# MarinerQ/npf_GWwaveform

Measured on AMD Instinct MI355X. Metric: waveform target-points/sec (train step), higher is better.
Workload: dtype f32 (every contraction of the step: fp32 operands as three exact bf16 terms, six v_mfma_f32_16x16x32_bf16 per product group, f32 accumulation -- f32 results, DESIGN.md 3.1 / 3.2; the 1-4-wide first / last layers: f32 FMAs); 1 GPU; BASELINE config 2: AttnCNP scaledot, r=256, 4-layer xy-encoder/decoder, 256 context / 1024 target points, 256 tasks per GPU (256 global), fp32 train step (fwd+loss+bwd+allreduce+Adam); tasks_per_gpu=256, global_tasks=256, context_points=256, target_points=1024, r_dim=256, n_params=799588, parallelism=dp1, hip_graph=True

## Files before the change

### npf_gwwaveform_amd/csrc/wgrad_kernel.hip

```cpp
#include "npf_common.hpp"

namespace npf {

constexpr int kWgThreads = 1024;
constexpr int kWgWaves = kWgThreads / 64;
constexpr int kWgMaxF = 256;
constexpr int kQRows = kWgMaxF / 4;
constexpr int kMaxJobs = 16;

struct WgradJobs {
  npf_wgrad_job_t job[kMaxJobs];
  int32_t first_wg[kMaxJobs + 1];
  int32_t n_jobs;
  int32_t n_tasks;
  int32_t tiles_per_task;
  int32_t pad;
  int64_t part_off[kMaxJobs];
};

__device__ __forceinline__ void wg_dma16(const float* src, float* lds_dst_wave_uniform) {
  __builtin_amdgcn_global_load_lds((const __attribute__((address_space(1))) void*)src,
                                   (__attribute__((address_space(3))) void*)lds_dst_wave_uniform, 16, 0, 0);
}

typedef __bf16 bf16x4 __attribute__((ext_vector_type(4)));
typedef __bf16 bf16x8w __attribute__((ext_vector_type(8)));
typedef __bf16 bf16x2v __attribute__((ext_vector_type(2)));
typedef float f32x2v __attribute__((ext_vector_type(2)));

__device__ __forceinline__ bf16x4 pack4_bf16(float a, float b, float c, float d) {
  const bf16x2v lo = __builtin_convertvector((f32x2v{a, b}), bf16x2v), hi = __builtin_convertvector((f32x2v{c, d}), bf16x2v);
  bf16x4 r;
  r[0] = lo[0]; r[1] = lo[1]; r[2] = hi[0]; r[3] = hi[1];
  return r;
}

__device__ __forceinline__ int wg_s0(int blk) { return 4 * (blk >> 1) + (blk & 1); }

__device__ __forceinline__ void operand16(const float* img, bool fmt16, int blk, int i, int g, int t2, bf16x4 (&op)[4],
                                          bool want_sum, f32x4& dsum) {
  if (!fmt16) {
    f32x4 q[4];
    const unsigned lbase = (unsigned)(size_t)(const __attribute__((address_space(3))) float*)img + (16 * blk + i) * 512;
#pragma unroll
    for (int jj = 0; jj < 4; ++jj) {
      const int c = 16 * t2 + 4 * g + jj;
      asm volatile("ds_read_b128 %0, %1" : "=v"(q[jj]) : "v"(lbase + ((c ^ i) << 4)));
    }
    asm volatile("s_waitcnt lgkmcnt(0)" : "+v"(q[0]), "+v"(q[1]), "+v"(q[2]), "+v"(q[3]));
    if (want_sum) dsum += (q[0] + q[1]) + (q[2] + q[3]);
#pragma unroll
    for (int m = 0; m < 4; ++m) op[m] = pack4_bf16(q[0][m], q[1][m], q[2][m], q[3][m]);
  } else {
    typedef unsigned u32x2 __attribute__((ext_vector_type(2)));
    const int q = i >> 2, p = i & 3;
    const int row0 = 4 * (wg_s0(blk) + 2 * (p >> 1));
    const int point = 16 * t2 + 4 * g + q;
    const unsigned base = (unsigned)(size_t)(const __attribute__((address_space(3))) float*)img + 8u * (p & 1);
    u32x2 r[4];
#pragma unroll
    for (int m = 0; m < 4; ++m) {
      const int row = row0 + m;
      asm volatile("ds_read_b64_tr_b16 %0, %1" : "=v"(r[m]) : "v"(base + row * 512 + ((point ^ (row & 15)) << 4)));
    }
    asm volatile("s_waitcnt lgkmcnt(0)" : "+v"(r[0]), "+v"(r[1]), "+v"(r[2]), "+v"(r[3]));
#pragma unroll
    for (int m = 0; m < 4; ++m) {
      op[m] = __builtin_bit_cast(bf16x4, r[m]);
    }
    if (want_sum) {
      f32x4 sm;
#pragma unroll
      for (int m = 0; m < 4; ++m)
        sm[m] = (__builtin_bit_cast(float, r[m][0] << 16) + __builtin_bit_cast(float, r[m][0] & 0xffff0000u)) +
                (__builtin_bit_cast(float, r[m][1] << 16) + __builtin_bit_cast(float, r[m][1] & 0xffff0000u));
      dsum += sm;
    }
  }
}

__device__ __forceinline__ int wg_feature(bool fmt16, int blk, int i, int m) {
  if (!fmt16) return 4 * (16 * blk + i) + m;
  return 32 * (wg_s0(blk) + 2 * (i >> 3)) + 16 * ((i >> 2) & 1) + 4 * m + (i & 3);
}
__device__ __forceinline__ bool wg_block_active(bool fmt16, int blk, int Fp) {
  return fmt16 ? 32 * wg_s0(blk) < Fp : 64 * blk < Fp;
}

template <bool BF16>
__global__ __launch_bounds__(kWgThreads, 4) void wgrad_kernel(const WgradJobs J, float* __restrict__ partials) {
  __shared__ __attribute__((aligned(16))) float lds[2 * 2 * kQRows * 128];
  constexpr int kOp = kQRows * 128;

  int j = 0;
  while (j + 1 < J.n_jobs && (int)blockIdx.x >= J.first_wg[j + 1]) ++j;
  const npf_wgrad_job_t& job = J.job[j];
  const int split = blockIdx.x - J.first_wg[j];
  const int n_split = J.first_wg[j + 1] - J.first_wg[j];
  const int Np = ((job.N + 31) >> 5) * 32, Kp = ((job.K + 31) >> 5) * 32;
  const long total_tiles = (long)J.n_tasks * J.tiles_per_task;
  long t0, t1;
  int tstride = 1;
  if (job.per_task) {
    t0 = (long)split * J.tiles_per_task;
    t1 = t0 + J.tiles_per_task;
  } else {
    t0 = split;
    t1 = total_tiles;
    tstride = n_split;
  }

  const int tid = threadIdx.x, lane = tid & 63;
  const int i = lane & 15, g = lane >> 4;
  const int wave = __builtin_amdgcn_readfirstlane(tid >> 6);
  const bool wide_rows = ((Kp + 63) >> 6) < ((Np + 63) >> 6);
  const int rg = wide_rows ? (wave & 3) : (wave >> 2);
  const int cg = wide_rows ? (wave >> 2) : (wave & 3);
  const bool act = wg_block_active(BF16 && (job.accumulate & NPF_WGRAD_DZ16) != 0, rg, Np) &&
                   wg_block_active(BF16 && (job.accumulate & NPF_WGRAD_A16) != 0, cg, Kp);

  for (int x = tid; x < 2 * 2 * kOp; x += kWgThreads) lds[x] = 0.f;

  const f32x4 zero4 = {0.f, 0.f, 0.f, 0.f};
  f32x4 acc[4][4];
#pragma unroll
  for (int m = 0; m < 4; ++m)
#pragma unroll
    for (int n = 0; n < 4; ++n) acc[m][n] = zero4;
  f32x4 dbacc = zero4;

  const unsigned dma_lane = 4u * (unsigned)((lane >> 5) * 128 + (((lane & 31) ^ ((2 * wave + (lane >> 5)) & 15)) << 2));
  const char* dz_base = (const char*)job.dZ;
  const char* a_base = (const char*)job.A;
  asm volatile("" : "+s"(dz_base), "+s"(a_base));
  const bool z16 = BF16 && (job.accumulate & NPF_WGRAD_DZ16) != 0, a16 = BF16 && (job.accumulate & NPF_WGRAD_A16) != 0;
  const int zsh = z16 ? 4 : 3, ash = a16 ? 4 : 3;
  const int Zf = job.ldz > 0 ? job.ldz : Np, Af = job.lda > 0 ? job.lda : Kp;
  auto tile_dma = [&](long t, float* buf) {
    const char* zsrc = dz_base + (((size_t)t * Zf) << (10 - zsh));
    const char* asrc = a_base + (((size_t)t * Af) << (10 - ash));
    for (int q = wave; q < (Np >> zsh); q += kWgWaves)
      wg_dma16((const float*)(zsrc + (size_t)q * 1024 + (size_t)dma_lane), buf + q * 256);
    for (int q = wave; q < (Kp >> ash); q += kWgWaves)
      wg_dma16((const float*)(asrc + (size_t)q * 1024 + (size_t)dma_lane), buf + kOp + q * 256);
  };

  [[maybe_unused]] const bool dual = z16 && a16;
  const long tstep = (BF16 && dual) ? 2 * (long)tstride : (long)tstride;
  auto step_dma = [&](long t, float* buf) {
    tile_dma(t, buf);
    if constexpr (BF16) {
      if (dual && t + tstride < t1) tile_dma(t + tstride, buf + kOp / 2);
    }
  };

  __syncthreads();
  if (t0 < t1 && !(BF16 && dual)) step_dma(t0, lds);

  unsigned za_l[4], ab_l[4];
  {
    const unsigned l0 = (unsigned)(size_t)(const __attribute__((address_space(3))) float*)lds;
#pragma unroll
    for (int t = 0; t < 4; ++t) {
      const unsigned lanepart = (((t ^ (i >> 2)) << 2) | (g ^ (i & 3))) << 4;
      za_l[t] = l0 + (16 * rg + i) * 512 + lanepart;
      ab_l[t] = l0 + kOp * 4 + (16 * cg + i) * 512 + lanepart;
    }
  }

  if constexpr (BF16) {
    if (dual) {
      const int pw = (wave < (Np >> zsh) ? 1 : 0) + (wave < (Kp >> ash) ? 1 : 0);
      auto slot_of = [&](long n) { return lds + ((n >> 1) & 1) * 2 * kOp + (n & 1) * (kOp / 2); };
      const long n_tiles = t0 < t1 ? (t1 - t0 + tstride - 1) / tstride : 0;
      for (long n = 0; n < 3 && n < n_tiles; ++n) tile_dma(t0 + n * tstride, slot_of(n));
      for (long n = 0; n < n_tiles; ++n) {
        const long younger = (n_tiles - 1 - n) < 2 ? (n_tiles - 1 - n) : 2;
        const int allow = (int)younger * pw;
        if (allow >= 4) asm volatile("s_waitcnt vmcnt(4)" ::: "memory");
        else if (allow >= 2) asm volatile("s_waitcnt vmcnt(2)" ::: "memory");
        else if (allow >= 1) asm volatile("s_waitcnt vmcnt(1)" ::: "memory");
        else asm volatile("s_waitcnt vmcnt(0)" ::: "memory");
        __builtin_amdgcn_s_barrier();
        if (n + 3 < n_tiles) tile_dma(t0 + (n + 3) * tstride, slot_of(n + 3));
        if (act) {
          const float* zimg = slot_of(n);
          const float* aimg = zimg + kOp;
          bf16x4 am[2][4], bn[2][4];
          f32x4 none = zero4;
          int iv = i, gv = g;
          asm volatile("" : "+v"(iv), "+v"(gv));
#pragma unroll
          for (int t2 = 0; t2 < 2; ++t2) {
            operand16(zimg, true, rg, iv, gv, t2, am[t2], cg == 0, dbacc);
            operand16(aimg, true, cg, iv, gv, t2, bn[t2], false, none);
          }
          bf16x8w a8[4], b8[4];
#pragma unroll
          for (int m = 0; m < 4; ++m) {
            a8[m] = __builtin_shufflevector(am[0][m], am[1][m], 0, 1, 2, 3, 4, 5, 6, 7);
            b8[m] = __builtin_shufflevector(bn[0][m], bn[1][m], 0, 1, 2, 3, 4, 5, 6, 7);
          }
#pragma unroll
          for (int m = 0; m < 4; ++m)
#pragma unroll
            for (int n2 = 0; n2 < 4; ++n2)
              acc[m][n2] = __builtin_amdgcn_mfma_f32_16x16x32_bf16(a8[m], b8[n2], acc[m][n2], 0, 0, 0);
        }
      }
      t0 = t1;
    }
  }
  int cur = 1;
  for (long t = t0; t < t1; t += tstep) {
    cur ^= 1;
    __syncthreads();
    if (t + tstep < t1) step_dma(t + tstep, lds + (cur ^ 1) * 2 * kOp);
    [[maybe_unused]] const unsigned boff = cur * 2 * kOp * 4;
    if constexpr (BF16) {
      const int nsub = (dual && t + tstride < t1) ? 2 : 1;
#pragma unroll 1
      for (int u = 0; act && u < nsub; ++u) {
        const float* zimg = lds + cur * 2 * kOp + u * (kOp / 2);
        const float* aimg = zimg + kOp;
#pragma unroll
        for (int t2 = 0; t2 < 2; ++t2) {
          bf16x4 am[4], bn[4];
          f32x4 none = zero4;
          int iv = i, gv = g;
          asm volatile("" : "+v"(iv), "+v"(gv));
          operand16(zimg, z16, rg, iv, gv, t2, am, cg == 0, dbacc);
          operand16(aimg, a16, cg, iv, gv, t2, bn, false, none);
#pragma unroll
          for (int m = 0; m < 4; ++m)
#pragma unroll
            for (int n2 = 0; n2 < 4; ++n2)
              acc[m][n2] = __builtin_amdgcn_mfma_f32_16x16x16bf16_1k(am[m], bn[n2], acc[m][n2], 0, 0, 0);
        }
      }
    } else if (act) {
      f32x4 fa[2], fb[2];
      asm volatile("ds_read_b128 %0, %2\n\tds_read_b128 %1, %3"
                   : "=&v"(fa[0]), "=&v"(fb[0])
                   : "v"(za_l[0] + boff), "v"(ab_l[0] + boff));
#pragma unroll
      for (int s = 0; s < 8; ++s) {
        const int c = s & 1, n = c ^ 1;
        if (s + 1 < 8) {
          asm volatile("s_waitcnt lgkmcnt(0)\n\tds_read_b128 %0, %4 offset:%6\n\tds_read_b128 %1, %5 offset:%6"
                       : "=&v"(fa[n]), "=&v"(fb[n]), "+v"(fa[c]), "+v"(fb[c])
                       : "v"(za_l[(s + 1) & 3] + boff), "v"(ab_l[(s + 1) & 3] + boff), "n"(((s + 1) >> 2) * 256));
        } else {
          asm volatile("s_waitcnt lgkmcnt(0)" : "+v"(fa[c]), "+v"(fb[c]));
        }
        if (cg == 0) dbacc += fa[c];
#pragma unroll
        for (int m = 0; m < 4; ++m)
#pragma unroll
          for (int n2 = 0; n2 < 4; ++n2)
            acc[m][n2] = __builtin_amdgcn_mfma_f32_16x16x4f32(fa[c][m], fb[c][n2], acc[m][n2], 0, 0, 0);
      }
    }
  }

  if (act) {
    int col[4];
#pragma unroll
    for (int n = 0; n < 4; ++n) col[n] = wg_feature(a16, cg, i, n);
    if (job.per_task) {
      const int Ko = job.ldo > 0 ? job.ldo : Kp;
      float* out = job.dW + (size_t)split * ((size_t)(Np >> 5) * Ko * 32);
#pragma unroll
      for (int m = 0; m < 4; ++m)
#pragma unroll
        for (int e = 0; e < 4; ++e) {
          const int row = wg_feature(z16, rg, 4 * g + e, m);
          if (row >= Np) continue;
          float* rbase = out + (size_t)(row >> 5) * (Ko >> 2) * 128 + (row & 31) * 4;
          if (!a16) {
            if (col[0] < Kp) {
              f32x4 v;
#pragma unroll
              for (int n = 0; n < 4; ++n) v[n] = acc[m][n][e];
              float* dst = rbase + (size_t)(col[0] >> 2) * 128;
              if (job.accumulate & NPF_WGRAD_ACCUMULATE) v += *(const f32x4*)dst;
              *(f32x4*)dst = v;
            }
          } else {
#pragma unroll
            for (int n = 0; n < 4; ++n)
              if (col[n] < Kp) {
                float* dst = rbase + (size_t)(col[n] >> 2) * 128 + (col[n] & 3);
                *dst = (job.accumulate & NPF_WGRAD_ACCUMULATE) ? *dst + acc[m][n][e] : acc[m][n][e];
              }
          }
        }
    } else {
      float* part = partials + J.part_off[j] + (size_t)split * ((size_t)Np * Kp + Np);
#pragma unroll
      for (int m = 0; m < 4; ++m)
#pragma unroll
        for (int e = 0; e < 4; ++e) {
          const int row = wg_feature(z16, rg, 4 * g + e, m);
          if (row >= Np) continue;
          if (!a16) {
            if (col[0] < Kp) {
              f32x4 v;
#pragma unroll
              for (int n = 0; n < 4; ++n) v[n] = acc[m][n][e];
              *(f32x4*)(part + (size_t)row * Kp + col[0]) = v;
            }
          } else {
#pragma unroll
            for (int n = 0; n < 4; ++n)
              if (col[n] < Kp) part[(size_t)row * Kp + col[n]] = acc[m][n][e];
          }
        }
      if (cg == 0) {
#pragma unroll
        for (int m = 0; m < 4; ++m) {
          dbacc[m] += __shfl_xor(dbacc[m], 16);
          dbacc[m] += __shfl_xor(dbacc[m], 32);
        }
        if (g == 0) {
          if (!z16) {
            if (wg_feature(false, rg, i, 0) < Np) *(f32x4*)(part + (size_t)Np * Kp + wg_feature(false, rg, i, 0)) = dbacc;
          } else {
#pragma unroll
            for (int m = 0; m < 4; ++m)
              if (wg_feature(true, rg, i, m) < Np) part[(size_t)Np * Kp + wg_feature(true, rg, i, m)] = dbacc[m];
          }
        }
      }
    }
  }
}

constexpr int kXThreads = 512;
constexpr int kXWaves = kXThreads / 64;

typedef float f32x8v __attribute__((ext_vector_type(8)));
struct X6Terms { bf16x8w t[3]; };

__device__ __forceinline__ unsigned x6_cvt_pk(float a, float b) {
  unsigned r;
  asm("v_cvt_pk_bf16_f32 %0, %1, %2" : "=v"(r) : "v"(a), "v"(b));
  return r;
}
__device__ __forceinline__ X6Terms x6_split(f32x8v v) {
  typedef unsigned u32x4v __attribute__((ext_vector_type(4)));
  u32x4v t0, t1, t2;
#pragma unroll
  for (int p = 0; p < 4; ++p) {
    const float a = v[2 * p], b = v[2 * p + 1];
    const unsigned h = x6_cvt_pk(a, b);
    const float ra = a - __builtin_bit_cast(float, h << 16), rb = b - __builtin_bit_cast(float, h & 0xffff0000u);
    const unsigned m = x6_cvt_pk(ra, rb);
    const float la = ra - __builtin_bit_cast(float, m << 16), lb = rb - __builtin_bit_cast(float, m & 0xffff0000u);
    t0[p] = h;
    t1[p] = m;
    t2[p] = x6_cvt_pk(la, lb);
  }
  X6Terms o;
  o.t[0] = __builtin_bit_cast(bf16x8w, t0);
  o.t[1] = __builtin_bit_cast(bf16x8w, t1);
  o.t[2] = __builtin_bit_cast(bf16x8w, t2);
  return o;
}

struct X6Raw { f32x4 q[8]; };
__device__ __forceinline__ void x6_issue(const unsigned (&ad)[4], X6Raw& r) {
  asm volatile("ds_read_b128 %0, %8\n\tds_read_b128 %1, %9\n\tds_read_b128 %2, %10\n\tds_read_b128 %3, %11\n\t"
               "ds_read_b128 %4, %8 offset:256\n\tds_read_b128 %5, %9 offset:256\n\t"
               "ds_read_b128 %6, %10 offset:256\n\tds_read_b128 %7, %11 offset:256"
               : "=&v"(r.q[0]), "=&v"(r.q[1]), "=&v"(r.q[2]), "=&v"(r.q[3]), "=&v"(r.q[4]), "=&v"(r.q[5]), "=&v"(r.q[6]),
                 "=&v"(r.q[7])
               : "v"(ad[0]), "v"(ad[1]), "v"(ad[2]), "v"(ad[3]));
}
struct X6Feat { float v[8]; };
template <int SEL>
__device__ __forceinline__ void x6_issue_feat(const unsigned (&ad)[4], X6Feat& r) {
  asm volatile("ds_read_b32 %0, %8 offset:%12\n\tds_read_b32 %1, %9 offset:%12\n\t"
               "ds_read_b32 %2, %10 offset:%12\n\tds_read_b32 %3, %11 offset:%12\n\t"
               "ds_read_b32 %4, %8 offset:%13\n\tds_read_b32 %5, %9 offset:%13\n\t"
               "ds_read_b32 %6, %10 offset:%13\n\tds_read_b32 %7, %11 offset:%13"
               : "=&v"(r.v[0]), "=&v"(r.v[1]), "=&v"(r.v[2]), "=&v"(r.v[3]), "=&v"(r.v[4]), "=&v"(r.v[5]), "=&v"(r.v[6]),
                 "=&v"(r.v[7])
               : "v"(ad[0]), "v"(ad[1]), "v"(ad[2]), "v"(ad[3]), "n"(SEL * 8192), "n"(SEL * 8192 + 256));
}
template <int N>
__device__ __forceinline__ void x6_wait_feat(X6Feat& r) {
  asm volatile("s_waitcnt lgkmcnt(%8)"
               : "+v"(r.v[0]), "+v"(r.v[1]), "+v"(r.v[2]), "+v"(r.v[3]), "+v"(r.v[4]), "+v"(r.v[5]), "+v"(r.v[6]), "+v"(r.v[7])
               : "n"(N));
}
__device__ __forceinline__ X6Terms x6_terms_of(const X6Feat& r) {
  return x6_split(f32x8v{r.v[0], r.v[1], r.v[2], r.v[3], r.v[4], r.v[5], r.v[6], r.v[7]});
}
__device__ __forceinline__ void x6_wait(X6Raw& r) {
  asm volatile("s_waitcnt lgkmcnt(0)"
               : "+v"(r.q[0]), "+v"(r.q[1]), "+v"(r.q[2]), "+v"(r.q[3]), "+v"(r.q[4]), "+v"(r.q[5]), "+v"(r.q[6]), "+v"(r.q[7]));
}
__device__ __forceinline__ X6Terms x6_terms_of(const X6Raw& r, int f) {
  const f32x8v v = {r.q[0][f], r.q[1][f], r.q[2][f], r.q[3][f], r.q[4][f], r.q[5][f], r.q[6][f], r.q[7][f]};
  return x6_split(v);
}

__global__ __launch_bounds__(kXThreads, 1) void wgrad_x6_kernel(const WgradJobs J, float* __restrict__ partials) {
  __shared__ __attribute__((aligned(16))) float lds[2 * 2 * kQRows * 128];
  constexpr int kOp = kQRows * 128;

  int j = 0;
  while (j + 1 < J.n_jobs && (int)blockIdx.x >= J.first_wg[j + 1]) ++j;
  const npf_wgrad_job_t& job = J.job[j];
  const int split = blockIdx.x - J.first_wg[j];
  const int n_split = J.first_wg[j + 1] - J.first_wg[j];
  const int Np = ((job.N + 31) >> 5) * 32, Kp = ((job.K + 31) >> 5) * 32;
  const long total_tiles = (long)J.n_tasks * J.tiles_per_task;
  long t0, t1;
  int tstride = 1;
  if (job.per_task) {
    t0 = (long)split * J.tiles_per_task;
    t1 = t0 + J.tiles_per_task;
  } else {
    t0 = split;
    t1 = total_tiles;
    tstride = n_split;
  }

  const int tid = threadIdx.x, lane = tid & 63;
  const int i = lane & 15, g = lane >> 4;
  const int wave = __builtin_amdgcn_readfirstlane(tid >> 6);
  const int rg = wave >> 1, cp = wave & 1;
  const bool act_r = 64 * rg < Np && 128 * cp < Kp;
  const int n_steps = !act_r ? 0 : (64 * (2 * cp + 1) < Kp ? 8 : 4);

  for (int x = tid; x < 2 * 2 * kOp; x += kXThreads) lds[x] = 0.f;

  const f32x4 zero4 = {0.f, 0.f, 0.f, 0.f};
  f32x4 acc[2][4][4];
#pragma unroll
  for (int c = 0; c < 2; ++c)
#pragma unroll
    for (int m = 0; m < 4; ++m)
#pragma unroll
      for (int n = 0; n < 4; ++n) acc[c][m][n] = zero4;
  f32x4 dbacc = zero4;

  const unsigned dma_lane = 4u * (unsigned)((lane >> 5) * 128 + (((lane & 31) ^ ((2 * wave + (lane >> 5)) & 15)) << 2));
  const char* dz_base = (const char*)job.dZ;
  const char* a_base = (const char*)job.A;
  asm volatile("" : "+s"(dz_base), "+s"(a_base));
  const int Zf = job.ldz > 0 ? job.ldz : Np, Af = job.lda > 0 ? job.lda : Kp;
  auto tile_dma = [&](long t, float* buf) {
    const char* zsrc = dz_base + (size_t)t * Zf * 128;
    const char* asrc = a_base + (size_t)t * Af * 128;
    for (int q = wave; q < (Np >> 3); q += kXWaves)
      wg_dma16((const float*)(zsrc + (size_t)q * 1024 + (size_t)dma_lane), buf + q * 256);
    for (int q = wave; q < (Kp >> 3); q += kXWaves)
      wg_dma16((const float*)(asrc + (size_t)q * 1024 + (size_t)dma_lane), buf + kOp + q * 256);
  };

  __syncthreads();
  if (t0 < t1) tile_dma(t0, lds);

  int cur = 1;
  for (long t = t0; t < t1; t += tstride) {
    cur ^= 1;
    __syncthreads();
    const bool dma_next = t + tstride < t1;
    float* nbuf = lds + (cur ^ 1) * 2 * kOp;
    if (n_steps == 0) {
      if (dma_next) tile_dma(t + tstride, nbuf);
      continue;
    }
    const char* zsrc_n = dz_base + (size_t)(t + tstride) * Zf * 128 + (size_t)dma_lane;
    const char* asrc_n = a_base + (size_t)(t + tstride) * Af * 128 + (size_t)dma_lane;
    int iv = i, gv = g;
    asm volatile("" : "+v"(iv), "+v"(gv));
    unsigned za[4], zb[4];
    {
      const unsigned l0 = (unsigned)(size_t)(const __attribute__((address_space(3))) float*)lds + cur * 2 * kOp * 4;
#pragma unroll
      for (int jj = 0; jj < 4; ++jj) {
        const unsigned lanepart = (unsigned)(((4 * gv + jj) ^ iv) << 4);
        za[jj] = l0 + (16 * rg + iv) * 512 + lanepart;
        zb[jj] = l0 + kOp * 4 + (32 * cp + iv) * 512 + lanepart;
      }
    }
    X6Raw ra;
    x6_issue(za, ra);
    x6_wait(ra);
    if (cp == 0) dbacc += ((ra.q[0] + ra.q[1]) + (ra.q[2] + ra.q[3])) + ((ra.q[4] + ra.q[5]) + (ra.q[6] + ra.q[7]));
    X6Terms fa[4];
#pragma unroll
    for (int m = 0; m < 4; ++m) fa[m] = x6_terms_of(ra, m);
    const unsigned pi4 = (unsigned)((iv >> 3) & 1) << 3;
    auto feat_addr = [&](int n2, unsigned (&ad)[4]) {
#pragma unroll
      for (int jj = 0; jj < 4; ++jj) ad[jj] = zb[jj] + ((4u * (unsigned)n2) ^ pi4);
    };
    X6Feat raw[2];
    {
      unsigned ad[4];
      feat_addr(0, ad);
      x6_issue_feat<0>(ad, raw[0]);
      feat_addr(1, ad);
      x6_issue_feat<0>(ad, raw[1]);
    }
    x6_wait_feat<8>(raw[0]);
    X6Terms fb = x6_terms_of(raw[0]);
#pragma unroll
    for (int k = 0; k < 8; ++k) {
      const int c = k >> 2, n2 = k & 3;
      if (dma_next) {
        const int q = wave + kXWaves * (k & 3);
        if (k < 4) {
          if (q < (Np >> 3)) wg_dma16((const float*)(zsrc_n + (size_t)q * 1024), nbuf + q * 256);
        } else {
          if (q < (Kp >> 3)) wg_dma16((const float*)(asrc_n + (size_t)q * 1024), nbuf + kOp + q * 256);
        }
      }
      if (k + 2 < 8) {
        unsigned ad[4];
        feat_addr((k + 2) & 3, ad);
        if (k + 2 < 4) x6_issue_feat<0>(ad, raw[k & 1]);
        else x6_issue_feat<1>(ad, raw[k & 1]);
      }
      X6Terms fb_next;
      if (k + 1 < 8) {
        if (k + 2 < 8) x6_wait_feat<8>(raw[(k + 1) & 1]);
        else x6_wait_feat<0>(raw[(k + 1) & 1]);
        fb_next = x6_terms_of(raw[(k + 1) & 1]);
      }
#pragma unroll
      for (int m = 0; m < 4; ++m) {
        f32x4 a = acc[c][m][n2];
        a = __builtin_amdgcn_mfma_f32_16x16x32_bf16(fa[m].t[2], fb.t[0], a, 0, 0, 0);
        a = __builtin_amdgcn_mfma_f32_16x16x32_bf16(fa[m].t[0], fb.t[2], a, 0, 0, 0);
        a = __builtin_amdgcn_mfma_f32_16x16x32_bf16(fa[m].t[1], fb.t[1], a, 0, 0, 0);
        a = __builtin_amdgcn_mfma_f32_16x16x32_bf16(fa[m].t[1], fb.t[0], a, 0, 0, 0);
        a = __builtin_amdgcn_mfma_f32_16x16x32_bf16(fa[m].t[0], fb.t[1], a, 0, 0, 0);
        a = __builtin_amdgcn_mfma_f32_16x16x32_bf16(fa[m].t[0], fb.t[0], a, 0, 0, 0);
        acc[c][m][n2] = a;
      }
      if (k + 1 < 8) {
#pragma unroll
        for (int q = 0; q < 24; ++q) {
          __builtin_amdgcn_sched_group_barrier(0x008, 1, 0);
          __builtin_amdgcn_sched_group_barrier(0x002, 2, 0);
        }
        fb = fb_next;
      }
    }
  }

#pragma unroll
  for (int c = 0; c < 2; ++c) {
    if (4 * c >= n_steps) continue;
    const int cg = 2 * cp + c;
    const int col0 = 4 * (16 * cg + i);
    if (job.per_task) {
      const int Ko = job.ldo > 0 ? job.ldo : Kp;
      float* out = job.dW + (size_t)split * ((size_t)(Np >> 5) * Ko * 32);
#pragma unroll
      for (int m = 0; m < 4; ++m)
#pragma unroll
        for (int e = 0; e < 4; ++e) {
          const int row = 4 * (16 * rg + 4 * g + e) + m;
          if (row >= Np || col0 >= Kp) continue;
          f32x4 v;
#pragma unroll
          for (int n = 0; n < 4; ++n) v[n] = (i & 8) ? acc[c][m][n ^ 2][e] : acc[c][m][n][e];
          float* dst = out + (size_t)(row >> 5) * (Ko >> 2) * 128 + (row & 31) * 4 + (size_t)(col0 >> 2) * 128;
          if (job.accumulate & NPF_WGRAD_ACCUMULATE) v += *(const f32x4*)dst;
          *(f32x4*)dst = v;
        }
    } else {
      float* part = partials + J.part_off[j] + (size_t)split * ((size_t)Np * Kp + Np);
#pragma unroll
      for (int m = 0; m < 4; ++m)
#pragma unroll
        for (int e = 0; e < 4; ++e) {
          const int row = 4 * (16 * rg + 4 * g + e) + m;
          if (row >= Np || col0 >= Kp) continue;
          f32x4 v;
#pragma unroll
          for (int n = 0; n < 4; ++n) v[n] = (i & 8) ? acc[c][m][n ^ 2][e] : acc[c][m][n][e];
          *(f32x4*)(part + (size_t)row * Kp + col0) = v;
        }
    }
  }
  if (!job.per_task && n_steps > 0 && cp == 0) {
    float* part = partials + J.part_off[j] + (size_t)split * ((size_t)Np * Kp + Np);
#pragma unroll
    for (int m = 0; m < 4; ++m) {
      dbacc[m] += __shfl_xor(dbacc[m], 16);
      dbacc[m] += __shfl_xor(dbacc[m], 32);
    }
    if (g == 0 && 4 * (16 * rg + i) < Np) *(f32x4*)(part + (size_t)Np * Kp + 4 * (16 * rg + i)) = dbacc;
  }
}

constexpr int kHRow = 576;
constexpr int kHTerm = 16 * kHRow;
constexpr int kHBuf = 2 * 3 * kHTerm;
typedef unsigned h16_u32x2 __attribute__((ext_vector_type(2)));
typedef unsigned h16_u32x4 __attribute__((ext_vector_type(4)));
typedef float f32x16v __attribute__((ext_vector_type(16)));

__global__ __launch_bounds__(512, 1) void wgrad_h16_kernel(const WgradJobs J, float* __restrict__ partials) {
  __shared__ __attribute__((aligned(16))) char lds[2 * kHBuf];
  int j = 0;
  while (j + 1 < J.n_jobs && (int)blockIdx.x >= J.first_wg[j + 1]) ++j;
  const npf_wgrad_job_t& job = J.job[j];
  const int split = blockIdx.x - J.first_wg[j];
  const int n_split = J.first_wg[j + 1] - J.first_wg[j];
  constexpr int Np = 256, Kp = 256;
  const long total_tiles = (long)J.n_tasks * J.tiles_per_task;
  long t0, t1;
  int tstride = 1;
  if (job.per_task) {
    t0 = (long)split * J.tiles_per_task;
    t1 = t0 + J.tiles_per_task;
  } else {
    t0 = split;
    t1 = total_tiles;
    tstride = n_split;
  }
  const long n_half = t1 > t0 ? 2 * ((t1 - t0 + tstride - 1) / tstride) : 0;

  const int tid = threadIdx.x, lane = tid & 63;
  const int wave = __builtin_amdgcn_readfirstlane(tid >> 6);
  const int rg = wave >> 1, cp = wave & 1;
  const int p_lo = lane & 3, q_ld = (lane >> 2) & 3, p_hi = lane >> 4;
  const int pt_ld = 4 * p_hi + p_lo;
  const int Zf = job.ldz > 0 ? job.ldz : Np, Af = job.lda > 0 ? job.lda : Kp;
  const char* dz_base = (const char*)job.dZ;
  const char* a_base = (const char*)job.A;
  const unsigned ld_lane = (unsigned)(((8 * wave + q_ld) * 32 + pt_ld) * 16);
  auto tile_of = [&](long h) { return t0 + (h >> 1) * tstride; };
  auto load_piece = [&](long h, int v) -> f32x4 {
    const long t = tile_of(h);
    const unsigned off = ld_lane + (unsigned)(h & 1) * 256u + (unsigned)(v & 1) * 2048u;
    const char* src = (v < 2 ? dz_base + (size_t)t * Zf * 128 : a_base + (size_t)t * Af * 128) + off;
    return *(const f32x4*)src;
  };
  const unsigned lds0 = (unsigned)(size_t)(__attribute__((address_space(3))) char*)lds;
  const unsigned st_lane = (unsigned)(pt_ld * kHRow + (8 * wave + q_ld) * 8);
  auto split_store1 = [&](const f32x4& x, int v, unsigned buf) {
    h16_u32x2 t[3];
#pragma unroll
    for (int pr = 0; pr < 2; ++pr) {
      const float a = x[2 * pr], b = x[2 * pr + 1];
      const unsigned h = x6_cvt_pk(a, b);
      const float ra = a - __builtin_bit_cast(float, h << 16), rb = b - __builtin_bit_cast(float, h & 0xffff0000u);
      const unsigned m = x6_cvt_pk(ra, rb);
      const float la = ra - __builtin_bit_cast(float, m << 16), lb = rb - __builtin_bit_cast(float, m & 0xffff0000u);
      t[0][pr] = h;
      t[1][pr] = m;
      t[2][pr] = x6_cvt_pk(la, lb);
    }
    const unsigned ad = lds0 + buf * kHBuf + (v >> 1) * 3 * kHTerm + st_lane + (v & 1) * 32;
    asm volatile("ds_write_b64 %0, %1\n\tds_write_b64 %0, %2 offset:%4\n\tds_write_b64 %0, %3 offset:%5"
                 :
                 : "v"(ad), "v"(t[0]), "v"(t[1]), "v"(t[2]), "n"(kHTerm), "n"(2 * kHTerm)
                 : "memory");
  };
  const int gq = lane >> 4, q_rd = (lane >> 2) & 3, p_rd = lane & 3;
  const unsigned rd_lane = (unsigned)((8 * (gq >> 1) + q_rd) * kHRow + (16 * (gq & 1) + 4 * p_rd) * 2);
  typedef short h16_s16x4 __attribute__((ext_vector_type(4)));
  typedef short h16_s16x8 __attribute__((ext_vector_type(8)));
  typedef __attribute__((address_space(3))) h16_s16x4 h16_lds_s16x4;
  struct Frag { h16_s16x8 v; };
  auto frag = [&](unsigned buf, int operand, int term, int feat0, Frag& f) {
    const char* ad = lds + buf * kHBuf + (operand * 3 + term) * kHTerm + rd_lane + (unsigned)feat0 * 2;
    const h16_s16x4 lo = __builtin_amdgcn_ds_read_tr16_b64_v4i16((h16_lds_s16x4*)ad);
    const h16_s16x4 hi = __builtin_amdgcn_ds_read_tr16_b64_v4i16((h16_lds_s16x4*)(ad + 4 * kHRow));
    f.v = __builtin_shufflevector(lo, hi, 0, 1, 2, 3, 4, 5, 6, 7);
  };
  auto op8 = [](const Frag& f) { return __builtin_bit_cast(bf16x8w, f.v); };

  f32x16v acc[2][4];
#pragma unroll
  for (int i = 0; i < 2; ++i)
#pragma unroll
    for (int c = 0; c < 4; ++c)
#pragma unroll
      for (int r = 0; r < 16; ++r) acc[i][c][r] = 0.f;
  f32x4 dbacc[2] = {f32x4{0.f, 0.f, 0.f, 0.f}, f32x4{0.f, 0.f, 0.f, 0.f}};

  f32x4 raw[4];
  auto body = [&](long h) {
    const unsigned buf = (unsigned)(h & 1);
    const float live = h + 1 < n_half ? 1.f : 0.f;
    const long h2 = h + 2 < n_half ? h + 2 : (n_half > 0 ? n_half - 1 : 0);
    Frag fa[2][3], fb[2][3];
#pragma unroll
    for (int i = 0; i < 2; ++i)
#pragma unroll
      for (int t = 0; t < 3; ++t) frag(buf, 0, t, 64 * rg + 32 * i, fa[i][t]);
#pragma unroll
    for (int t = 0; t < 3; ++t) frag(buf, 1, t, 128 * cp, fb[0][t]);
#pragma unroll
    for (int c = 0; c < 4; ++c) {
      const int cb = c & 1;
      if (c + 1 < 4) {
#pragma unroll
        for (int t = 0; t < 3; ++t) frag(buf, 1, t, 128 * cp + 32 * (c + 1), fb[cb ^ 1][t]);
      }
#define HMM(I, TA, TB) \
  acc[I][c] = __builtin_amdgcn_mfma_f32_32x32x16_bf16(op8(fa[I][TA]), op8(fb[cb][TB]), acc[I][c], 0, 0, 0)
      HMM(0, 2, 0);
      HMM(1, 2, 0);
      HMM(0, 0, 2);
      HMM(1, 0, 2);
      HMM(0, 1, 1);
      HMM(1, 1, 1);
      HMM(0, 1, 0);
      HMM(1, 1, 0);
      HMM(0, 0, 1);
      HMM(1, 0, 1);
      HMM(0, 0, 0);
      HMM(1, 0, 0);
#undef HMM
      if (c < 2) dbacc[c] += raw[c] * live;
      split_store1(raw[c], c, buf ^ 1);
      raw[c] = load_piece(h2, c);
#pragma unroll
      for (int q = 0; q < 12; ++q) {
        __builtin_amdgcn_sched_group_barrier(0x008, 1, 0);
        __builtin_amdgcn_sched_group_barrier(0x002, 2, 0);
      }
    }
    __syncthreads();
  };

  if (n_half > 0) {
#pragma unroll
    for (int v = 0; v < 4; ++v) raw[v] = load_piece(0, v);
    dbacc[0] += raw[0];
    dbacc[1] += raw[1];
#pragma unroll
    for (int v = 0; v < 4; ++v) split_store1(raw[v], v, 0);
#pragma unroll
    for (int v = 0; v < 4; ++v) raw[v] = load_piece(n_half > 1 ? 1 : 0, v);
  }
  __syncthreads();
  for (long h = 0; h < n_half; ++h) body(h);

  const int col_l = lane & 31, row_l = 4 * (lane >> 5);
  if (job.per_task) {
    const int Ko = job.ldo > 0 ? job.ldo : Kp;
    float* out = job.dW + (size_t)split * ((size_t)(Np >> 5) * Ko * 32);
#pragma unroll
    for (int i = 0; i < 2; ++i)
#pragma unroll
      for (int c = 0; c < 4; ++c)
#pragma unroll
        for (int r = 0; r < 16; ++r) {
          const int row = 64 * rg + 32 * i + (r & 3) + 8 * (r >> 2) + row_l, col = 128 * cp + 32 * c + col_l;
          float* dst = out + (size_t)(row >> 5) * (Ko >> 2) * 128 + (row & 31) * 4 + (size_t)(col >> 2) * 128 + (col & 3);
          *dst = (job.accumulate & NPF_WGRAD_ACCUMULATE) ? *dst + acc[i][c][r] : acc[i][c][r];
        }
  } else {
    float* part = partials + J.part_off[j] + (size_t)split * ((size_t)Np * Kp + Np);
#pragma unroll
    for (int i = 0; i < 2; ++i)
#pragma unroll
      for (int c = 0; c < 4; ++c)
#pragma unroll
        for (int r = 0; r < 16; ++r) {
          const int row = 64 * rg + 32 * i + (r & 3) + 8 * (r >> 2) + row_l, col = 128 * cp + 32 * c + col_l;
          part[(size_t)row * Kp + col] = acc[i][c][r];
        }
#pragma unroll
    for (int v = 0; v < 2; ++v) {
#pragma unroll
      for (int e = 0; e < 4; ++e) {
        float x = dbacc[v][e];
        x += __shfl_xor(x, 1);
        x += __shfl_xor(x, 2);
        x += __shfl_xor(x, 16);
        x += __shfl_xor(x, 32);
        dbacc[v][e] = x;
      }
      if (pt_ld == 0) *(f32x4*)(part + (size_t)Np * Kp + 4 * (8 * wave + 4 * v + q_ld)) = dbacc[v];
    }
  }
}

__global__ void wgrad_reduce_kernel(const WgradJobs J, const float* __restrict__ partials) {
  const int j = blockIdx.y;
  const npf_wgrad_job_t& job = J.job[j];
  if (job.per_task) return;
  const int n_split = J.first_wg[j + 1] - J.first_wg[j];
  const int Np = ((job.N + 31) >> 5) * 32, Kp = ((job.K + 31) >> 5) * 32;
  const size_t slab = (size_t)Np * Kp + Np;
  const float* part = partials + J.part_off[j];
  const int total4 = (Np * Kp + Np) >> 2;
  for (int i4 = blockIdx.x * blockDim.x + threadIdx.x; i4 < total4; i4 += gridDim.x * blockDim.x) {
    const float* p = part + (size_t)i4 * 4;
    f32x4 s0 = {0.f, 0.f, 0.f, 0.f}, s1 = s0, s2 = s0, s3 = s0;
    int sp = 0;
    for (; sp + 4 <= n_split; sp += 4) {
      s0 += *(const f32x4*)(p + (size_t)sp * slab);
      s1 += *(const f32x4*)(p + (size_t)(sp + 1) * slab);
      s2 += *(const f32x4*)(p + (size_t)(sp + 2) * slab);
      s3 += *(const f32x4*)(p + (size_t)(sp + 3) * slab);
    }
    for (; sp < n_split; ++sp) s0 += *(const f32x4*)(p + (size_t)sp * slab);
    const f32x4 s = (s0 + s1) + (s2 + s3);
    const int idx = i4 * 4;
    if (idx < Np * Kp) {
      const int n = idx / Kp, k = idx - n * Kp;
      if (n < job.N) {
        float* d = job.dW + (size_t)n * job.ldw + k;
#pragma unroll
        for (int e = 0; e < 4; ++e)
          if (k + e < job.K) d[e] = (job.accumulate & NPF_WGRAD_ACCUMULATE) ? d[e] + s[e] : s[e];
      }
    } else if (job.db) {
      const int n = idx - Np * Kp;
#pragma unroll
      for (int e = 0; e < 4; ++e)
        if (n + e < job.N) job.db[n + e] = (job.accumulate & NPF_WGRAD_ACCUMULATE) ? job.db[n + e] + s[e] : s[e];
    }
  }
}

static int plan(const npf_wgrad_job_t* jobs, int n_jobs, int n_tasks, int tiles_per_task, WgradJobs* J) {
  if (!jobs || n_jobs <= 0 || n_jobs > kMaxJobs || n_tasks <= 0 || tiles_per_task <= 0) return NPF_EINVAL;
  const long total_tiles = (long)n_tasks * tiles_per_task;
  int n_shared = 0;
  for (int j = 0; j < n_jobs; ++j) {
    const npf_wgrad_job_t& b = jobs[j];
    if (!b.dZ || !b.A || !b.dW || b.N <= 0 || b.K <= 0 || b.N > npf::kWgMaxF || b.K > npf::kWgMaxF) return NPF_EINVAL;
    if ((((uintptr_t)b.dZ) | ((uintptr_t)b.A)) & 15) return NPF_EINVAL;
    if (b.per_task && (((uintptr_t)b.dW) & 15)) return NPF_EINVAL;
    if (!b.per_task && b.ldw < b.K) return NPF_EINVAL;
    if (b.ldz < 0 || b.lda < 0 || b.ldo < 0 || (b.ldz & 31) || (b.lda & 31) || (b.ldo & 31)) return NPF_EINVAL;
    if ((b.ldz && b.ldz < npf::round_up(b.N, 32)) || (b.lda && b.lda < npf::round_up(b.K, 32)) ||
        (b.ldo && b.ldo < npf::round_up(b.K, 32)))
      return NPF_EINVAL;
    n_shared += b.per_task ? 0 : 1;
  }
  bool bf16 = true, x6 = true;
  for (int j = 0; j < n_jobs; ++j) {
    bf16 &= (jobs[j].accumulate & NPF_WGRAD_BF16) != 0;
    x6 &= (jobs[j].accumulate & (NPF_WGRAD_F32X6 | NPF_WGRAD_BF16)) == NPF_WGRAD_F32X6;
  }
  double cost[kMaxJobs], cost_sum = 0.0;
  for (int j = 0; j < n_jobs; ++j) {
    const int Np = npf::round_up(jobs[j].N, 32), Kp = npf::round_up(jobs[j].K, 32);
    const int ar = (Np + 63) / 64, ac = (Kp + 63) / 64;
    const double zb = (jobs[j].accumulate & NPF_WGRAD_DZ16) ? 2.0 : 4.0, ab = (jobs[j].accumulate & NPF_WGRAD_A16) ? 2.0 : 4.0;
    const double bytes = 32.0 * (Np * zb + Kp * ab);
    if (jobs[j].per_task) cost[j] = 0.0;
    else if (bf16) cost[j] = bytes > 18432.0 ? bytes : 18432.0;
    else if (x6) {
      const int waves = ar * ((ac + 1) / 2);
      const double mf = 3072.0 * 1.6 * ((waves + 3) / 4) + 2500.0, mem = bytes / 6.5;
      cost[j] = mf > mem ? mf : mem;
    } else {
      const double mf = 4096.0 * (ar < ac ? ar : ac), mem = bytes / 6.5;
      cost[j] = mf > mem ? mf : mem;
    }
    cost_sum += cost[j];
  }
  J->n_jobs = n_jobs;
  J->n_tasks = n_tasks;
  J->tiles_per_task = tiles_per_task;
  J->pad = 0;
  long splits_of[kMaxJobs];
  long used = 0;
  for (int j = 0; j < n_jobs; ++j) {
    splits_of[j] = 0;
    if (jobs[j].per_task) continue;
    long sp = (long)(256.0 * cost[j] / cost_sum);
    if (sp < 1) sp = 1;
    if (sp > total_tiles) sp = total_tiles;
    splits_of[j] = sp;
    used += sp;
  }
  for (int j = 0; j < n_jobs && used < 256; ++j)
    if (!jobs[j].per_task && cost[j] * n_shared >= cost_sum && splits_of[j] < total_tiles) {
      ++splits_of[j];
      ++used;
    }
  int wg = 0;
  int64_t off = 0;
  for (int j = 0; j < n_jobs; ++j) {
    J->job[j] = jobs[j];
    J->first_wg[j] = wg;
    J->part_off[j] = off;
    if (jobs[j].per_task) {
      wg += n_tasks;
    } else {
      const int Np = npf::round_up(jobs[j].N, 32), Kp = npf::round_up(jobs[j].K, 32);
      const long splits = splits_of[j];
      wg += (int)splits;
      off += (int64_t)splits * ((int64_t)Np * Kp + Np);
    }
  }
  J->first_wg[n_jobs] = wg;
  for (int j = n_jobs + 1; j <= kMaxJobs; ++j) J->first_wg[j] = wg;
  return (int)0;
}

}

extern "C" int64_t npf_wgrad_partials_bytes(const npf_wgrad_job_t* jobs, int32_t n_jobs, int32_t n_tasks,
                                            int32_t tiles_per_task) {
  npf::WgradJobs J;
  if (npf::plan(jobs, n_jobs, n_tasks, tiles_per_task, &J) != 0) return -1;
  int64_t off = 0;
  for (int j = 0; j < n_jobs; ++j) {
    if (jobs[j].per_task) continue;
    const int Np = npf::round_up(jobs[j].N, 32), Kp = npf::round_up(jobs[j].K, 32);
    off += (int64_t)(J.first_wg[j + 1] - J.first_wg[j]) * ((int64_t)Np * Kp + Np);
  }
  return off * 4 + 16;
}

extern "C" int npf_wgrad_run(const npf_wgrad_job_t* jobs, int32_t n_jobs, int32_t n_tasks, int32_t tiles_per_task,
                             float* partials, int64_t partials_bytes, void* stream) {
  npf::WgradJobs J;
  const int rc = npf::plan(jobs, n_jobs, n_tasks, tiles_per_task, &J);
  if (rc != 0) return rc;
  const int64_t need = npf_wgrad_partials_bytes(jobs, n_jobs, n_tasks, tiles_per_task);
  bool any_shared = false;
  for (int j = 0; j < n_jobs; ++j) any_shared |= !jobs[j].per_task;
  if (any_shared && (!partials || partials_bytes < need || (((uintptr_t)partials) & 15))) return NPF_EINVAL;
  const int n_wg = J.first_wg[n_jobs];
  bool bf16 = true, x6 = true;
  for (int j = 0; j < n_jobs; ++j) {
    bf16 &= (jobs[j].accumulate & NPF_WGRAD_BF16) != 0;
    x6 &= (jobs[j].accumulate & (NPF_WGRAD_F32X6 | NPF_WGRAD_BF16)) == NPF_WGRAD_F32X6;
  }
  bool h16 = x6;
  for (int j = 0; j < n_jobs; ++j) h16 &= jobs[j].N == 256 && jobs[j].K == 256 && !(jobs[j].accumulate & NPF_WGRAD_NO_H16);
  if (h16)
    hipLaunchKernelGGL(npf::wgrad_h16_kernel, dim3(n_wg), dim3(512), 0, (hipStream_t)stream, J, partials);
  else if (x6)
    hipLaunchKernelGGL(npf::wgrad_x6_kernel, dim3(n_wg), dim3(npf::kXThreads), 0, (hipStream_t)stream, J, partials);
  else if (bf16)
    hipLaunchKernelGGL(npf::wgrad_kernel<true>, dim3(n_wg), dim3(npf::kWgThreads), 0, (hipStream_t)stream, J, partials);
  else
    hipLaunchKernelGGL(npf::wgrad_kernel<false>, dim3(n_wg), dim3(npf::kWgThreads), 0, (hipStream_t)stream, J, partials);
  NPF_CHECK_LAUNCH();
  if (any_shared) {
    hipLaunchKernelGGL(npf::wgrad_reduce_kernel, dim3(65, n_jobs), dim3(256), 0, (hipStream_t)stream, J,
                       (const float*)partials);
    NPF_CHECK_LAUNCH();
  }
  return NPF_OK;
}
```

Baseline: 43.48 million target-points/s.

## Software-pipeline wgrad fragment loads across tiles and stage per-task output via LDS

Restructures the wgrad main loop so the first A/B fragments of the next half-tile are read from LDS right after the barrier and overlap the last MFMA group, using ping-pong fragment registers and a two-step unrolled loop. The store/load of the raw pieces is rebalanced across the first three column groups, and the syncthreads is replaced by an explicit lgkmcnt wait plus s_barrier. The per-task output path now stages accumulators in LDS per wave and writes coalesced 16-byte vectors instead of scattered scalar stores. The extra fragment registers raise register pressure, and the unroll by two assumes n_half is even or relies on clamped tails.

Result: no change. 43.81 million target-points/s (median of 6 runs) (+0.8%).

```diff
diff --git a/npf_gwwaveform_amd/csrc/wgrad_kernel.hip b/npf_gwwaveform_amd/csrc/wgrad_kernel.hip
--- a/npf_gwwaveform_amd/csrc/wgrad_kernel.hip
+++ b/npf_gwwaveform_amd/csrc/wgrad_kernel.hip
@@ -646,7 +646,6 @@
     const char* src = (v < 2 ? dz_base + (size_t)t * Zf * 128 : a_base + (size_t)t * Af * 128) + off;
     return *(const f32x4*)src;
   };
-  const unsigned lds0 = (unsigned)(size_t)(__attribute__((address_space(3))) char*)lds;
   const unsigned st_lane = (unsigned)(pt_ld * kHRow + (8 * wave + q_ld) * 8);
   auto split_store1 = [&](const f32x4& x, int v, unsigned buf) {
     h16_u32x2 t[3];
@@ -661,11 +660,12 @@
       t[1][pr] = m;
       t[2][pr] = x6_cvt_pk(la, lb);
     }
-    const unsigned ad = lds0 + buf * kHBuf + (v >> 1) * 3 * kHTerm + st_lane + (v & 1) * 32;
-    asm volatile("ds_write_b64 %0, %1\n\tds_write_b64 %0, %2 offset:%4\n\tds_write_b64 %0, %3 offset:%5"
-                 :
-                 : "v"(ad), "v"(t[0]), "v"(t[1]), "v"(t[2]), "n"(kHTerm), "n"(2 * kHTerm)
-                 : "memory");
+    typedef __attribute__((address_space(3))) h16_u32x2 h16_lds_u32x2;
+    h16_lds_u32x2* ad = (h16_lds_u32x2*)((__attribute__((address_space(3))) char*)lds + buf * kHBuf + (v >> 1) * 3 * kHTerm +
+                                         st_lane + (v & 1) * 32);
+    ad[0] = t[0];
+    ad[kHTerm / 8] = t[1];
+    ad[2 * kHTerm / 8] = t[2];
   };
   const int gq = lane >> 4, q_rd = (lane >> 2) & 3, p_rd = lane & 3;
   const unsigned rd_lane = (unsigned)((8 * (gq >> 1) + q_rd) * kHRow + (16 * (gq & 1) + 4 * p_rd) * 2);
@@ -691,49 +691,62 @@
   f32x4 dbacc[2] = {f32x4{0.f, 0.f, 0.f, 0.f}, f32x4{0.f, 0.f, 0.f, 0.f}};
 
   f32x4 raw[4];
-  auto body = [&](long h) {
-    const unsigned buf = (unsigned)(h & 1);
+  Frag fA[2][3], fB[2][3], fb[2][3];
+  auto first_frags = [&](unsigned buf, Frag (&f)[2][3]) {
+#pragma unroll
+    for (int i = 0; i < 2; ++i)
+#pragma unroll
+      for (int t = 0; t < 3; ++t) frag(buf, 0, t, 64 * rg + 32 * i, f[i][t]);
+#pragma unroll
+    for (int t = 0; t < 3; ++t) frag(buf, 1, t, 128 * cp, fb[0][t]);
+  };
+  auto body = [&](long h, unsigned buf, Frag (&fa)[2][3], Frag (&fn)[2][3]) {
     const float live = h + 1 < n_half ? 1.f : 0.f;
     const long h2 = h + 2 < n_half ? h + 2 : (n_half > 0 ? n_half - 1 : 0);
-    Frag fa[2][3], fb[2][3];
-#pragma unroll
-    for (int i = 0; i < 2; ++i)
-#pragma unroll
-      for (int t = 0; t < 3; ++t) frag(buf, 0, t, 64 * rg + 32 * i, fa[i][t]);
-#pragma unroll
-    for (int t = 0; t < 3; ++t) frag(buf, 1, t, 128 * cp, fb[0][t]);
-#pragma unroll
-    for (int c = 0; c < 4; ++c) {
-      const int cb = c & 1;
-      if (c + 1 < 4) {
-#pragma unroll
-        for (int t = 0; t < 3; ++t) frag(buf, 1, t, 128 * cp + 32 * (c + 1), fb[cb ^ 1][t]);
-      }
 #define HMM(I, TA, TB) \
   acc[I][c] = __builtin_amdgcn_mfma_f32_32x32x16_bf16(op8(fa[I][TA]), op8(fb[cb][TB]), acc[I][c], 0, 0, 0)
-      HMM(0, 2, 0);
-      HMM(1, 2, 0);
-      HMM(0, 0, 2);
-      HMM(1, 0, 2);
-      HMM(0, 1, 1);
-      HMM(1, 1, 1);
-      HMM(0, 1, 0);
-      HMM(1, 1, 0);
-      HMM(0, 0, 1);
-      HMM(1, 0, 1);
-      HMM(0, 0, 0);
-      HMM(1, 0, 0);
-#undef HMM
-      if (c < 2) dbacc[c] += raw[c] * live;
-      split_store1(raw[c], c, buf ^ 1);
-      raw[c] = load_piece(h2, c);
+#define HMM12() \
+  HMM(0, 2, 0); HMM(1, 2, 0); HMM(0, 0, 2); HMM(1, 0, 2); HMM(0, 1, 1); HMM(1, 1, 1); \
+  HMM(0, 1, 0); HMM(1, 1, 0); HMM(0, 0, 1); HMM(1, 0, 1); HMM(0, 0, 0); HMM(1, 0, 0)
+#pragma unroll
+    for (int c = 0; c < 3; ++c) {
+      const int cb = c & 1;
+#pragma unroll
+      for (int t = 0; t < 3; ++t) frag(buf, 1, t, 128 * cp + 32 * (c + 1), fb[cb ^ 1][t]);
+      HMM12();
+      if (c == 0) {
+#pragma unroll
+        for (int v = 0; v < 2; ++v) {
+          dbacc[v] += raw[v] * live;
+          split_store1(raw[v], v, buf ^ 1);
+          raw[v] = load_piece(h2, v);
+        }
+      } else {
+        split_store1(raw[c + 1], c + 1, buf ^ 1);
+        raw[c + 1] = load_piece(h2, c + 1);
+      }
 #pragma unroll
       for (int q = 0; q < 12; ++q) {
         __builtin_amdgcn_sched_group_barrier(0x008, 1, 0);
-        __builtin_amdgcn_sched_group_barrier(0x002, 2, 0);
-      }
-    }
-    __syncthreads();
+        if (c == 0) __builtin_amdgcn_sched_group_barrier(0x002, 5, 0);
+        else __builtin_amdgcn_sched_group_barrier(0x002, 3, 0);
+      }
+    }
+    __builtin_amdgcn_sched_barrier(0);
+    asm volatile("s_waitcnt lgkmcnt(0)\n\ts_barrier" ::: "memory");
+    __builtin_amdgcn_sched_barrier(0);
+    {
+      constexpr int c = 3, cb = 1;
+      first_frags(buf ^ 1, fn);
+      HMM12();
+#pragma unroll
+      for (int q = 0; q < 9; ++q) {
+        __builtin_amdgcn_sched_group_barrier(0x008, 1, 0);
+        __builtin_amdgcn_sched_group_barrier(0x100, 2, 0);
+      }
+    }
+#undef HMM12
+#undef HMM
   };
 
   if (n_half > 0) {
@@ -747,22 +760,38 @@
     for (int v = 0; v < 4; ++v) raw[v] = load_piece(n_half > 1 ? 1 : 0, v);
   }
   __syncthreads();
-  for (long h = 0; h < n_half; ++h) body(h);
+  first_frags(0, fA);
+  for (long h = 0; h < n_half; h += 2) {
+    body(h, 0, fA, fB);
+    body(h + 1, 1, fB, fA);
+  }
+  __syncthreads();
 
   const int col_l = lane & 31, row_l = 4 * (lane >> 5);
   if (job.per_task) {
     const int Ko = job.ldo > 0 ? job.ldo : Kp;
     float* out = job.dW + (size_t)split * ((size_t)(Np >> 5) * Ko * 32);
+    constexpr int kQuad = 132;
+    float* stage = (float*)lds + wave * (8 * kQuad);
+    const int st_w = (col_l >> 2) * kQuad + row_l * 4 + (col_l & 3);
 #pragma unroll
     for (int i = 0; i < 2; ++i)
 #pragma unroll
-      for (int c = 0; c < 4; ++c)
-#pragma unroll
-        for (int r = 0; r < 16; ++r) {
-          const int row = 64 * rg + 32 * i + (r & 3) + 8 * (r >> 2) + row_l, col = 128 * cp + 32 * c + col_l;
-          float* dst = out + (size_t)(row >> 5) * (Ko >> 2) * 128 + (row & 31) * 4 + (size_t)(col >> 2) * 128 + (col & 3);
-          *dst = (job.accumulate & NPF_WGRAD_ACCUMULATE) ? *dst + acc[i][c][r] : acc[i][c][r];
-        }
+      for (int c = 0; c < 4; ++c) {
+#pragma unroll
+        for (int r = 0; r < 16; ++r) stage[st_w + ((r & 3) + 8 * (r >> 2)) * 4] = acc[i][c][r];
+        __builtin_amdgcn_wave_barrier();
+        float* tile = out + (size_t)(2 * rg + i) * (Ko >> 2) * 128 + (size_t)(32 * cp + 8 * c) * 128;
+#pragma unroll
+        for (int k = 0; k < 4; ++k) {
+          const int quad = 2 * k + (lane >> 5);
+          f32x4 v = *(const f32x4*)(stage + quad * kQuad + (lane & 31) * 4);
+          float* dst = tile + 256 * k + 4 * lane;
+          if (job.accumulate & NPF_WGRAD_ACCUMULATE) v += *(const f32x4*)dst;
+          *(f32x4*)dst = v;
+        }
+        __builtin_amdgcn_wave_barrier();
+      }
   } else {
     float* part = partials + J.part_off[j] + (size_t)split * ((size_t)Np * Kp + Np);
 #pragma unroll
```
